# CRIPAC-DIG/GET

Measured on AMD Instinct MI355X. Metric: claim-evidence pairs/sec fwd+bwd (B=32, h=300), higher is better.
Workload: dtype f32

## Files before the change

get_amd/csrc/cell_ops.hip:

```cpp
#include "../../include/get_hip.h"
#include "gemm_batch.h"
#include "common.h"

using namespace gh;

int gh::cell_fwd_impl(int bf, float* out32, const uint64_t* bits, const float* dinv, const float* vals, const uint64_t* keep,
                                const int32_t* goff, int m_real, int m_rows,
                                const float* x, const int32_t* ids, int n, int r, int din, int h,
                                const float* w_p, const float* w_z0, const float* w_z1, const float* w_r0,
                                const float* w_r1, const float* w_h0, const float* w_h1,
                                const float* b_z0, const float* b_z1, const float* b_r0, const float* b_r1,
                                const float* b_h0, const float* b_h1,
                                float* xp, float* a, float* z, float* rr, float* rx, float* hh, float* out,
                                float drop_p, uint32_t drop_seed,
                                const float* score_w, float* score_x, float score_drop_p, uint32_t score_drop_seed,
                                gh_stream_t stream, int pad_out_dead, int* score_parts, float* xdrop) {
  hipStream_t s = (hipStream_t)stream;
  if (score_parts) *score_parts = 1;
  GH_REQUIRE(n > 0 && r > 0 && din > 0 && h > 0, "ggnn_cell_fwd: bad sizes n=%d r=%d din=%d h=%d", n, r, din, h);
  GH_REQUIRE(!bf || (din % 8 == 0 && h % 8 == 0), "ggnn_cell_fwd_bf16: needs din %% 8 == 0, h %% 8 == 0 (din=%d h=%d)", din, h);
  if (!goff) { m_real = n * r; m_rows = n * r; }
  GH_REQUIRE(m_real >= 0 && m_real <= m_rows && m_rows <= n * r, "ggnn_cell_fwd: node-compact rows %d/%d do not fit n*r=%d", m_real, m_rows, n * r);
  const int M = m_rows;
  if (M == 0) return 0;
// ... 102 lines not shown
                       score_x, score_drop_p, score_drop_seed, stream, 0, nullptr, nullptr);
}

extern "C" int gh_ggnn_cell_fwd_bf16(const uint64_t* bits, const float* dinv, const float* vals, const uint64_t* keep,
                                     const int32_t* goff, int m_real, int m_rows,
                                     const void* x, const int32_t* ids, int n, int r, int din, int h,
                                     const void* w_p, const void* w_z0, const void* w_z1, const void* w_r0,
                                     const void* w_r1, const void* w_h0, const void* w_h1,
                                     const float* b_z0, const float* b_z1, const float* b_r0, const float* b_r1,
                                     const float* b_h0, const float* b_h1,
                                     void* xp, void* a, void* z, void* rr, void* rx, void* hh, void* out, float* out32,
                                     float drop_p, uint32_t drop_seed,
                                     const float* score_w, float* score_x, float score_drop_p, uint32_t score_drop_seed,
                                     gh_stream_t stream) {
  typedef const float* cf;
  typedef float* mf;
  return cell_fwd_impl(1, out32, bits, dinv, vals, keep, goff, m_real, m_rows, (cf)x, ids, n, r, din, h, (cf)w_p, (cf)w_z0, (cf)w_z1,
                       (cf)w_r0, (cf)w_r1, (cf)w_h0, (cf)w_h1, b_z0, b_z1, b_r0, b_r1, b_h0, b_h1, (mf)xp, (mf)a, (mf)z, (mf)rr,
                       (mf)rx, (mf)hh, (mf)out, drop_p, drop_seed, score_w, score_x, score_drop_p, score_drop_seed, stream, 0, nullptr, nullptr);
}

int gh::cell_bwd_impl(int bf, const uint64_t* bits, const float* dinv, const float* vals, const uint64_t* keep,
                                const int32_t* goff, int m_real,
                                const float* x, const int32_t* ids, int n, int r, int din, int h,
                                const float* wt_p, const float* wt_z0, const float* wt_z1, const float* wt_r0,
                                const float* wt_r1, const float* wt_h0, const float* wt_h1,
                                const float* xp, const float* a, const float* z, const float* rr, const float* rx,
                                const float* hh, const float* g,
                                float* dhp, float* dzp, float* drp, float* dxp, float* da,
                                float* dx, float* dw_p, float* dw_z0, float* dw_z1, float* dw_r0, float* dw_r1,
                                float* dw_h0, float* dw_h1, float* db_z, float* db_r, float* db_h,
                                float* db_z1, float* db_r1, float* db_h1, float drop_p, uint32_t drop_seed,
                                gh_stream_t stream, gh_stream_t wstream, hipEvent_t ev_l1, hipEvent_t ev_agg,
                                int pre_done, const GateFuse* next, const float* xdrop) {
  hipStream_t s = (hipStream_t)stream;
  hipStream_t sw = wstream ? (hipStream_t)wstream : s;
  const bool two = sw != s;
  GH_REQUIRE(!two || (ev_l1 && ev_agg), "ggnn_cell_bwd: a separate weight-gradient stream needs its two events");
  GH_REQUIRE(n > 0 && r > 0 && din > 0 && h > 0, "ggnn_cell_bwd: bad sizes");
  GH_REQUIRE(!bf || (din % 8 == 0 && h % 8 == 0 && din <= h), "ggnn_cell_bwd_bf16: needs din %% 8 == 0, h %% 8 == 0, din <= h (din=%d h=%d)", din, h);
  if (!goff) m_real = n * r;
  GH_REQUIRE(m_real >= 0 && m_real <= n * r, "ggnn_cell_bwd: node-compact rows %d do not fit n*r=%d", m_real, n * r);
  GH_REQUIRE(drop_p <= 0.f || (long long)n * r * (long long)din < (1LL << 32),
             "ggnn_cell_bwd: %d rows x %d columns exceed the dropout mask's 32-bit element index", n * r, din);
  const int M = m_real;
  if (M == 0) return 0;
  if (!pre_done)
    if (int e = launch_gate_bwd_pre(g, z, hh, xp, dhp, dzp, dxp, (size_t)M * h, s, bf)) return e;
  const bool wide = bf && h % 256 == 0;
  {
    Batch b(false, M, s, wide, SITE_CELL_BWD_H, h);
    Problem p0 = gemm_problem(M, h, EPI_STORE, da, h, dhp, h, wt_h0, h, h, nullptr, bf);
    Problem p1 = gemm_problem(M, h, EPI_BWD_DRX, drp, h, dhp, h, wt_h1, h, h, nullptr, bf);
    p1.out1 = dxp; p1.in0 = xp; p1.in1 = rr;
    p0.io = bf ? 1 : 0; p1.io = bf ? 15 : 0;
    b.add(p0); b.add(p1);
    b.flush();
    GH_CHECK_HIP(b.err);
  }
  const bool cs = bf ? true : (h % 4 == 0);
  auto add_gate_wgrads = [&](Batch& b) {
    b.add(tn_problem(h, h, dw_z0, h, dzp, h, a, h, M, nullptr, bf));  if (cs) b.want_colsum(db_z, db_z1);
    b.add(tn_problem(h, h, dw_z1, h, dzp, h, xp, h, M, nullptr, bf));
    b.add(tn_problem(h, h, dw_r0, h, drp, h, a, h, M, nullptr, bf));  if (cs) b.want_colsum(db_r, db_r1);
    b.add(tn_problem(h, h, dw_r1, h, drp, h, xp, h, M, nullptr, bf));
    b.add(tn_problem(h, h, dw_h0, h, dhp, h, a, h, M, nullptr, bf));  if (cs) b.want_colsum(db_h, db_h1);
    b.add(tn_problem(h, h, dw_h1, h, dhp, h, rx, h, M, nullptr, bf));
  };
  bool colsum_done = false;
  if (two) {
    GH_CHECK_HIP(hipEventRecord(ev_l1, s));
    GH_CHECK_HIP(hipStreamWaitEvent(sw, ev_l1, 0));
    Batch b(true, M, sw);
    add_gate_wgrads(b);
    b.flush();
    GH_CHECK_HIP(b.err);
    colsum_done = b.colsum_fused && !b.colsum_missed;
    if (!colsum_done) {
      GH_REQUIRE(!bf, "ggnn_cell_bwd_bf16: the bias gradients need the split-K workspace (gh_set_workspace)");
      if (int e = launch_colsum3(dzp, drp, dhp, db_z, db_r, db_h, M, h, sw, db_z1, db_r1, db_h1)) return e;
    }
  }
// ... 32 lines not shown
    Batch b(true, M, sw);
    if (!two) add_gate_wgrads(b);
    if (bf && xdrop && drop_p > 0.f && din <= h) {
      b.add(tn_problem(h, din, dw_p, din, dxp, h, xdrop, din, M, nullptr, bf));
    } else if ((ids || drop_p > 0.f || bf) && din <= h) {
      if (int e = launch_gather_rows(x, ids, da, M, din, sw, drop_p, drop_seed, bf)) return e;
      b.add(tn_problem(h, din, dw_p, din, dxp, h, da, din, M, nullptr, bf));
    } else {
      GH_REQUIRE(drop_p == 0.f, "ggnn_cell_bwd: fused dropout needs din (%d) <= h (%d)", din, h);
      b.add(tn_problem(h, din, dw_p, din, dxp, h, x, din, M, ids));
    }
    b.flush();
    GH_CHECK_HIP(b.err);
    if (two || (b.colsum_fused && !b.colsum_missed)) return 0;
  }
  GH_REQUIRE(!bf, "ggnn_cell_bwd_bf16: the bias gradients need the split-K workspace (gh_set_workspace)");
  return launch_colsum3(dzp, drp, dhp, db_z, db_r, db_h, M, h, s, db_z1, db_r1, db_h1);
}

extern "C" int gh_ggnn_cell_bwd(const uint64_t* bits, const float* dinv, const float* vals, const uint64_t* keep,
                                const int32_t* goff, int m_real,
                                const float* x, const int32_t* ids, int n, int r, int din, int h,
                                const float* wt_p, const float* wt_z0, const float* wt_z1, const float* wt_r0,
                                const float* wt_r1, const float* wt_h0, const float* wt_h1,
                                const float* xp, const float* a, const float* z, const float* rr, const float* rx,
                                const float* hh, const float* g,
                                float* dhp, float* dzp, float* drp, float* dxp, float* da,
                                float* dx, float* dw_p, float* dw_z0, float* dw_z1, float* dw_r0, float* dw_r1,
                                float* dw_h0, float* dw_h1, float* db_z, float* db_r, float* db_h,
                                float* db_z1, float* db_r1, float* db_h1, float drop_p, uint32_t drop_seed,
                                gh_stream_t stream) {
  return cell_bwd_impl(0, bits, dinv, vals, keep, goff, m_real, x, ids, n, r, din, h, wt_p, wt_z0, wt_z1, wt_r0, wt_r1, wt_h0, wt_h1,
                       xp, a, z, rr, rx, hh, g, dhp, dzp, drp, dxp, da, dx, dw_p, dw_z0, dw_z1, dw_r0, dw_r1, dw_h0, dw_h1,
                       db_z, db_r, db_h, db_z1, db_r1, db_h1, drop_p, drop_seed, stream, nullptr, nullptr, nullptr, 0, nullptr, nullptr);
}

extern "C" int gh_ggnn_cell_bwd_bf16(const uint64_t* bits, const float* dinv, const float* vals, const uint64_t* keep,
                                     const int32_t* goff, int m_real,
                                     const void* x, const int32_t* ids, int n, int r, int din, int h,
                                     const void* wt_p, const void* wt_z0, const void* wt_z1, const void* wt_r0,
                                     const void* wt_r1, const void* wt_h0, const void* wt_h1,
                                     const void* xp, const void* a, const void* z, const void* rr, const void* rx,
                                     const void* hh, const float* g,
                                     void* dhp, void* dzp, void* drp, void* dxp, void* da,
                                     float* dx, float* dw_p, float* dw_z0, float* dw_z1, float* dw_r0, float* dw_r1,
                                     float* dw_h0, float* dw_h1, float* db_z, float* db_r, float* db_h,
                                     float* db_z1, float* db_r1, float* db_h1, float drop_p, uint32_t drop_seed,
                                     gh_stream_t stream) {
  typedef const float* cf;
  typedef float* mf;
  return cell_bwd_impl(1, bits, dinv, vals, keep, goff, m_real, (cf)x, ids, n, r, din, h, (cf)wt_p, (cf)wt_z0, (cf)wt_z1, (cf)wt_r0,
                       (cf)wt_r1, (cf)wt_h0, (cf)wt_h1, (cf)xp, (cf)a, (cf)z, (cf)rr, (cf)rx, (cf)hh, g, (mf)dhp, (mf)dzp, (mf)drp,
                       (mf)dxp, (mf)da, dx, dw_p, dw_z0, dw_z1, dw_r0, dw_r1, dw_h0, dw_h1, db_z, db_r, db_h, db_z1, db_r1,
                       db_h1, drop_p, drop_seed, stream, nullptr, nullptr, nullptr, 0, nullptr, nullptr);
}
```

get_amd/csrc/common.h:

```cpp
#pragma once
#include <hip/hip_runtime.h>
#include <stdint.h>
#include <stdio.h>
#include <stdlib.h>
#include <string.h>

namespace gh {

void set_error(const char* fmt, ...);

#define GH_CHECK_HIP(expr)                                                                  \
  do {                                                                                      \
    hipError_t _e = (expr);                                                                 \
    if (_e != hipSuccess) {                                                                 \
      gh::set_error("%s:%d: %s -> %s", __FILE__, __LINE__, #expr, hipGetErrorString(_e));   \
      return 1;                                                                             \
    }                                                                                       \
  } while (0)

#define GH_REQUIRE(cond, ...)                     \
  do {                                            \
    if (!(cond)) {                                \
      gh::set_error(__VA_ARGS__);                 \
      return 2;                                   \
// ... 68 lines not shown
int launch_att_softmax_bwd(const float* right, const float* weights, const float* g_att, const float* g_w,
                           const int32_t* goff, int m_real, int b, int l, int dr, int heads, float* de, float* dright,
                           hipStream_t s, const int32_t* rowg = nullptr, float* dw_tmp = nullptr, int* dw_written = nullptr,
                           const void* right16 = nullptr);
int launch_att_dpre(const float* de, const float* w2, const float* t, const int32_t* goff, int m_real, int b, int l,
                    int ha, int heads, float* dpre, float* du, float* dw2_part, hipStream_t s, const float* dw_in = nullptr,
                    const float* weights = nullptr, float* de_out = nullptr, void* dpre16 = nullptr,
                    long long dw_range_stride = 0, int dw_ranges = 1);

struct Workspace { float* p; size_t bytes; float* cs; size_t cs_bytes; };
Workspace workspace_for(hipStream_t s);
int gemm_mode();

struct GateFuse { const float* z; const float* hh; const float* xp; float* dhp; float* dzp; float* dxp; int bf16; };

int cell_fwd_impl(int bf, float* out32, const uint64_t* bits, const float* dinv, const float* vals, const uint64_t* keep,
                  const int32_t* goff, int m_real, int m_rows, const float* x, const int32_t* ids, int n, int r, int din, int h,
                  const float* w_p, const float* w_z0, const float* w_z1, const float* w_r0, const float* w_r1, const float* w_h0,
                  const float* w_h1, const float* b_z0, const float* b_z1, const float* b_r0, const float* b_r1, const float* b_h0,
                  const float* b_h1, float* xp, float* a, float* z, float* rr, float* rx, float* hh, float* out, float drop_p,
                  uint32_t drop_seed, const float* score_w, float* score_x, float score_drop_p, uint32_t score_drop_seed,
                  void* stream, int pad_out_dead = 0,
                  int* score_parts = nullptr,
                  float* xdrop = nullptr);
int cell_bwd_impl(int bf, const uint64_t* bits, const float* dinv, const float* vals, const uint64_t* keep, const int32_t* goff,
                  int m_real, const float* x, const int32_t* ids, int n, int r, int din, int h, const float* wt_p,
                  const float* wt_z0, const float* wt_z1, const float* wt_r0, const float* wt_r1, const float* wt_h0,
                  const float* wt_h1, const float* xp, const float* a, const float* z, const float* rr, const float* rx,
                  const float* hh, const float* g, float* dhp, float* dzp, float* drp, float* dxp, float* da, float* dx,
                  float* dw_p, float* dw_z0, float* dw_z1, float* dw_r0, float* dw_r1, float* dw_h0, float* dw_h1, float* db_z,
                  float* db_r, float* db_h, float* db_z1, float* db_r1, float* db_h1, float drop_p, uint32_t drop_seed, void* stream,
                  void* wstream, hipEvent_t ev_l1, hipEvent_t ev_agg,
                  int pre_done, const GateFuse* next,
                  const float* xdrop = nullptr);
int att_fwd_impl(const float* left, int nl, const int32_t* rowu, const float* right, const float* mask, const int32_t* goff,
                 const int32_t* rowg, int m_real, int b, int l, int xl, int dr, int ha, int heads, const float* w1, const float* w2,
                 float* u, float* t, float* e, float* weights, float* attended, hipStream_t s, int u_mode = 0,
                 const void* right16 = nullptr, const void* w1_16 = nullptr);
int att_bwd_impl(const float* left, const float* right, const int32_t* goff, int m_real, int b, int l, int xl, int dr, int ha,
                 int heads, const float* w1t, const float* w2, const float* t, const float* weights, const float* g_att,
                 const float* g_w, float* de, float* dpre, float* du, float* dleft, float* dright, float* dw1, float* dw2,
                 const int32_t* claim_offsets, int nl, float* du_c, int dleft_accumulate, hipStream_t s,
                 const int32_t* rowg = nullptr, float* dw_tmp = nullptr, const GateFuse* next = nullptr, int dleft_late = 0,
                 float* dw2_buf = nullptr, const void* right16 = nullptr, const void* w1t_16 = nullptr);
int linear2_fwd(const float* x0, int k0, const float* x1, int k1, const float* w, const float* bias, float* y, int m, int n, hipStream_t s,
                const float* w_out = nullptr, const float* b_out = nullptr, float* y_out = nullptr, int n_out = 0);
int linear2_bwd(const float* x0, int k0, const float* x1, int k1, const float* wt, const float* g, int m, int n, float* dx0,
                int dx0_accumulate, float* dx1, float* dw, float* db, hipStream_t s);

}
```

get_amd/csrc/gemm_batch.h:

```cpp
#pragma once
#include "common.h"
#include "gemm.hip.h"

namespace gh {

enum BatchSite : int {
  SITE_NONE = 0,
  SITE_CELL_ZR = 1,
  SITE_CELL_H = 2,
  SITE_CELL_BWD_H = 3,
  SITE_CELL_BWD_ZR = 4,
  SITE_CELL_BWD_DX = 5,
  SITE_ATT_BWD_DRIGHT = 6,
  SITE_CELL_PROJ = 7,
};
constexpr int NARROW_DEFAULT = 14;

long long generic_launches();

struct Batch {
  Batch(bool tn, int rows_hint, hipStream_t s, bool wide_bf16 = false, int site = SITE_NONE, int n_hint = 0);
  void add(const Problem& p);
  void flush();
  void want_colsum(float* o, float* o2) { if (L.nprob > 0) { cs_out[L.nprob - 1] = o; cs_out2[L.nprob - 1] = o2; } }

  int bm, bn;
  hipError_t err = hipSuccess;
  bool colsum_fused = false;
  bool colsum_missed = false;
  bool split_done = false;
  float* g_ws = nullptr;
  size_t g_ws_bytes = 0;
  bool narrow = false;
  long long e_block_stride = 0;

 private:
  Launch L;
  bool tn, big;
  hipStream_t s;
  int k_total = 0;
  float* cs_out[GH_MAX_PROBLEMS] = {nullptr};
  float* cs_out2[GH_MAX_PROBLEMS] = {nullptr};
  bool wide = false;
  bool wide256 = false;
  bool tn_pp = false;
  bool tn_pp_ok(const Problem& p) const;
  void reset();
  hipError_t launch_any();
  bool nt_split_plan();
};

int launch_att_finish(float* t, const float* u, const float* w2, float* e, const int32_t* urow, int M, int ha, int l, int heads, hipStream_t s);
int launch_reduce_wave(const float* parts, int n_parts, float* out, int I, int J, hipStream_t s);

inline Problem gemm_problem(int M, int N, int epi, float* C, int ldc, const float* A, int lda, const float* B, int ldb,
                            int K, const int32_t* gatherA = nullptr, int elt = 0) {
  Problem p = make_problem(M, N, epi, C, ldc);
  p.elt = elt;
  p.seg[0] = make_seg_nt(A, lda, B, ldb, K, gatherA, elt);
  return p;
}
inline void add_seg(Problem& p, const float* A, int lda, const float* B, int ldb, int K) {
  p.seg[p.nseg++] = make_seg_nt(A, lda, B, ldb, K, nullptr, p.elt);
}
inline void set_dropout(Problem& p, int mode, int ld, float drop_p, unsigned seed) {
  if (drop_p <= 0.f) return;
  p.drop_mode = mode; p.drop_ld = ld; p.drop_col0 = 0; p.drop_seed = seed;
  const double t = (double)drop_p * 4294967296.0;
  p.drop_thresh = t >= 4294967295.0 ? 4294967295u : (unsigned)t;
  p.drop_scale = 1.0f / (1.0f - drop_p);
}
inline Problem tn_problem(int I, int J, float* C, int ldc, const float* A, int lda, const float* B, int ldb, int K,
                          const int32_t* gatherB = nullptr, int elt = 0) {
  Problem p = make_problem(I, J, EPI_ATOMIC, C, ldc);
  p.seg[0] = make_seg_tn(A, lda, I, B, ldb, J, K, nullptr, gatherB);
  p.elt = elt;
  if (elt) {
    p.seg[0].vecA = ((reinterpret_cast<uintptr_t>(A) & 15) == 0) && lda % 8 == 0 && I % 8 == 0;
    p.seg[0].vecB = ((reinterpret_cast<uintptr_t>(B) & 15) == 0) && ldb % 8 == 0 && J % 8 == 0;
  }
  return p;
}

}
```

get_amd/csrc/gemm_ops.hip:

```cpp
#include "../../include/get_hip.h"
#include "gemm_batch.h"
#include "device_utils.h"
#include "gemm_nt.hip.h"
#include "gemm_tn.hip.h"
#include "gemm_tn_pp.hip.h"
#include <stdlib.h>

namespace gh {

static bool s_lds_bad(const Problem& p) { return p.seg[0].lda % 8 || p.seg[0].ldb % 8; }
static void fast_why(int rule, int prob, const Problem* p = nullptr, int seg = -1) {
  static const bool dbg = measure_env("GH_FASTOK_DEBUG", 0) != 0;
  if (!dbg) return;
  fprintf(stderr, "gemm: generic kernel (fast_ok rule %d, problem %d)\n", rule, prob);
  if (p && seg >= 0) fprintf(stderr, "   seg %d lda %d M %d N %d K %d\n", seg, p->seg[seg].lda, p->M, p->N, p->seg[seg].K);
}
static bool fast_ok(const Launch& L, bool tn) {
  for (int i = 0; i < L.nprob; ++i) {
    const Problem& p = L.p[i];
    const int ns = tn ? 1 : p.nseg;
    for (int j = 0; j < ns; ++j) {
      const Seg& s = p.seg[j];
      if (!s.vecA || !s.vecB || s.gatherB || s.K < 4) { fast_why(1, i); return false; }
      if (tn && s.gatherA) { fast_why(2, i); return false; }
// ... 294 lines not shown
      for (int u = 0; u < 8; ++u) v[u] = *reinterpret_cast<const float4*>(p + (size_t)(k + u) * it.stride);
#pragma unroll
      for (int u = 0; u < 8; ++u) { acc.x += v[u].x; acc.y += v[u].y; acc.z += v[u].z; acc.w += v[u].w; }
    }
    for (; k < it.ks; ++k) {
      const float4 v = *reinterpret_cast<const float4*>(p + (size_t)k * it.stride);
      acc.x += v.x; acc.y += v.y; acc.z += v.z; acc.w += v.w;
    }
    float* o = it.out + (size_t)i * it.ldc + j;
    o[0] += acc.x; o[1] += acc.y; o[2] += acc.z; o[3] += acc.w;
  }
}

__global__ void __launch_bounds__(256)
reduce_partials_wave_kernel(const ReduceArgs R) {
  const ReduceItem& it = R.it[blockIdx.y];
  const int J4 = it.J / 4;
  const int total = it.I * J4;
  const int e = blockIdx.x * 4 + (threadIdx.x >> 6), lane = threadIdx.x & 63;
  if (e >= total) return;
  const int i = e / J4, j = 4 * (e % J4);
  const float* p = it.ws + (size_t)i * it.J + j;
  float4 acc = make_float4(0.f, 0.f, 0.f, 0.f);
  for (int k = lane; k < it.ks; k += 64) {
    const float4 v = *reinterpret_cast<const float4*>(p + (size_t)k * it.stride);
    acc.x += v.x; acc.y += v.y; acc.z += v.z; acc.w += v.w;
  }
  for (int o = 32; o > 0; o >>= 1) {
    acc.x += __shfl_xor(acc.x, o); acc.y += __shfl_xor(acc.y, o); acc.z += __shfl_xor(acc.z, o); acc.w += __shfl_xor(acc.w, o);
  }
  if (lane == 0) {
    float* o = it.out + (size_t)i * it.ldc + j;
    o[0] += acc.x; o[1] += acc.y; o[2] += acc.z; o[3] += acc.w;
  }
}

struct FinishItem {
  const float* ws; long long stride; int ks; int M, N, epi, accumulate, ldc;
  float* C; const float* bias; const float* bias2; float* out1; const float* in0; const float* in1;
  const float* u; const float* w2; float* e; int ldu, R, heads;
  const int32_t* rowg;
};

struct FinishArgs { FinishItem it[GH_MAX_PROBLEMS]; int n; int split; };

__global__ void __launch_bounds__(256)
nt_finish_kernel(const FinishArgs F) {
  const FinishItem& it = F.it[blockIdx.y];
  const int lane = threadIdx.x & 63, wave = threadIdx.x >> 6;
  const bool split = F.split != 0;
  const int row = split ? (int)blockIdx.x : (int)blockIdx.x * 4 + wave;
  if (row >= it.M) return;
  const int N4 = it.N / 4;
  __shared__ float4 part[3][64];
  int kb = 0, ke = it.ks;
  if (split) { const int kq = (it.ks + 3) / 4; kb = wave * kq; ke = min(it.ks, kb + kq); }
  float pe[8];
#pragma unroll
  for (int c = 0; c < 8; ++c) pe[c] = 0.f;
  for (int c0 = 0; c0 < N4; c0 += 64) {
    const int c4 = c0 + lane;
    const int col = 4 * c4;
    float4 v = make_float4(0.f, 0.f, 0.f, 0.f);
    if (c4 < N4 && kb < ke) {
      const float* p = it.ws + (size_t)row * it.N + col;
      for (int k0 = kb; k0 < ke; k0 += 8) {
// ... 317 lines not shown
    q.split_stride = (long long)q.M * q.N;
    w += (size_t)ks * q.M * q.N;
    if (q.M > max_m) max_m = q.M;
  }
  L.ksplit = ks;
  L.kchunk = ct * 16;
  hipError_t e = launch_any();
  if (e != hipSuccess) err = e;
  F.split = (ks >= 16 && max_m <= 8192) ? 1 : 0;
  hipLaunchKernelGGL(nt_finish_kernel, dim3(F.split ? max_m : (max_m + 3) / 4, F.n), dim3(256), 0, s, F);
  split_done = true;
  e = hipGetLastError();
  if (e != hipSuccess) err = e;
  reset();
  return true;
}

int launch_att_finish(float* t, const float* u, const float* w2, float* e, const int32_t* urow, int M, int ha, int l, int heads, hipStream_t s) {
  FinishArgs F;
  F.n = 1; F.split = 0;
  F.it[0] = FinishItem{t, 0, 1, M, ha, EPI_ATT, 0, ha, t, nullptr, nullptr, nullptr, nullptr, nullptr, u, w2, e, ha, l, heads, urow};
  hipLaunchKernelGGL(nt_finish_kernel, dim3((M + 3) / 4, 1), dim3(256), 0, s, F);
  GH_LAUNCH_CHECK();
  return 0;
}
int launch_reduce_wave(const float* parts, int n_parts, float* out, int I, int J, hipStream_t s) {
  ReduceArgs R;
  R.n = 1;
  R.it[0] = ReduceItem{parts, out, I, J, J, n_parts, (long long)I * J};
  hipLaunchKernelGGL(reduce_partials_wave_kernel, dim3((I * (J / 4) + 3) / 4, 1), dim3(256), 0, s, R);
  GH_LAUNCH_CHECK();
  return 0;
}

}

using namespace gh;

extern "C" int gh_set_gemm_mode(int mode) {
  GH_REQUIRE(mode >= 0 && mode <= 3, "set_gemm_mode: %d is not 0 (fp32), 1 (bf16 operands in the big NT/NN GEMMs), 2 (fp32x3) or 3 (fp32x3, pre-split weights)", mode);
  g_gemm_mode = mode;
  return 0;
}

extern "C" int gh_weights_changed(void) {
  std::lock_guard<std::mutex> lk(g_x3_mu);
  ++g_x3_epoch;
  return 0;
}

extern "C" int gh_fp32x3_refresh(gh_stream_t stream) {
  std::lock_guard<std::mutex> lk(g_x3_mu);
  if (g_x3.empty()) return 0;
  std::vector<X3Item> items;
  items.reserve(g_x3.size());
  for (auto& kv : g_x3) {
    items.push_back(X3Item{(const float*)kv.first.b, kv.second.img, kv.first.N, kv.first.ldb, kv.first.K, kv.second.pitch});
    kv.second.epoch = g_x3_epoch;
  }
  x3p_split(items.data(), (int)items.size(), (hipStream_t)stream);
  GH_CHECK_HIP(hipGetLastError());
  return 0;
}

extern "C" int gh_fp32x3_clear(void) {
  std::lock_guard<std::mutex> lk(g_x3_mu);
// ... 40 lines not shown
```

get_amd/csrc/model_ops.hip:

```cpp
#include "../../include/get_hip.h"
#include "common.h"
#include <mutex>
#include <unordered_map>

namespace gh {

struct Dims {
  int B, B1, L, R, n, D, H, hw, he, C, cs, as, Xl, Xa, Dre, E, W;
  bool compact;
  int Mr, Mt, M1, Mq;
  bool bf;
  bool att16;
  bool fuse_scorer;
};
struct CellBuf { int64_t xp, a, z, rr, rx, hh, out, out32, xdrop; };
struct FwdBuf {
  int64_t offsets, pair2claim, has, lens_eff, rowc, maskf_p;
  CellBuf q, c1, c2;
  int64_t q_repr, score_x, score, keep;
  int64_t uw, tw, ew, ww, avg, new_left;
  int64_t right_e, mask_e, ue, te, ee, we, att_e, y0, phi;
  int64_t total;
  int64_t obs_total;
};
// ... 271 lines not shown
  P->phi = f.phi; P->word_w = f.ww; P->evd_w = f.we; P->score = f.score; P->keep = f.keep;
  return 0;
}

extern "C" int gh_get_struct_sizes(int64_t* out) {
  GH_REQUIRE(out, "get_struct_sizes: NULL");
  out[0] = sizeof(gh_get_model); out[1] = sizeof(gh_get_batch); out[2] = sizeof(gh_get_plan); out[3] = sizeof(gh_cell_params);
  out[4] = sizeof(gh_cell_bf16);
  return 0;
}

#define GH_TRY(expr) do { if (int _rc = (expr)) return _rc; } while (0)

static inline const int32_t* I32(const float* A, int64_t off) { return reinterpret_cast<const int32_t*>(A + off); }
static inline int32_t* I32(float* A, int64_t off) { return reinterpret_cast<int32_t*>(A + off); }

static int cell_fwd(const gh_cell_params& c, const gh_cell_bf16* c16, const CellBuf& cb, float* A, const uint64_t* bits, const float* dinv,
                    const float* vals, const uint64_t* keep, const int32_t* goff, int m_real, int m_rows, const float* x, const int32_t* ids,
                    int n, int r, int din, int h, float drop_p, uint32_t seed, const float* score_w, float* score_x, float sdrop,
                    uint32_t sseed, hipStream_t s, int pad_out_dead = 0, int* score_parts = nullptr) {
  typedef const float* cf;
  if (c16)
    return cell_fwd_impl(1, cb.out32 >= 0 ? A + cb.out32 : nullptr, bits, dinv, vals, keep, goff, m_real, m_rows, x, ids, n, r, din, h, (cf)c16->w_p, (cf)c16->w_z0,
                         (cf)c16->w_z1, (cf)c16->w_r0, (cf)c16->w_r1, (cf)c16->w_h0, (cf)c16->w_h1, c.b_z0, c.b_z1, c.b_r0, c.b_r1, c.b_h0,
                         c.b_h1, A + cb.xp, A + cb.a, A + cb.z, A + cb.rr, A + cb.rx, A + cb.hh, A + cb.out, drop_p, seed, score_w, score_x,
                         sdrop, sseed, (void*)s, 0, score_parts, cb.xdrop >= 0 ? A + cb.xdrop : nullptr);
  return cell_fwd_impl(0, nullptr, bits, dinv, vals, keep, goff, m_real, m_rows, x, ids, n, r, din, h, c.w_p, c.w_z0, c.w_z1, c.w_r0,
                       c.w_r1, c.w_h0, c.w_h1, c.b_z0, c.b_z1, c.b_r0, c.b_r1, c.b_h0, c.b_h1, A + cb.xp, A + cb.a, A + cb.z,
                       A + cb.rr, A + cb.rx, A + cb.hh, A + cb.out, drop_p, seed, score_w, score_x, sdrop, sseed, (void*)s, pad_out_dead);
}
static int cell_bwd(const gh_cell_params& c, const gh_cell_bf16* c16, const CellBuf& cb, const float* A, const uint64_t* bits, const float* dinv,
                    const float* vals, const uint64_t* keep, const int32_t* goff, int m_real, const float* x, const int32_t* ids, int n,
                    int r, int din, int h, const float* g, float* W, const int64_t* sc, float* dx, float drop_p, uint32_t seed,
                    hipStream_t s, int pre_done = 0, const GateFuse* next = nullptr) {
  GH_REQUIRE(c.dw_p && c.db_z0 && c.db_z1, "get_backward: a cell's gradient outputs are missing");
  if (c16) {
    typedef const float* cf;
    GH_REQUIRE(c16->wt_p && c16->wt_z0 && c16->wt_z1 && c16->wt_r0 && c16->wt_r1 && c16->wt_h0 && c16->wt_h1,
               "get_backward: storage = 1 needs the bf16 twins of the cells' transposed weights (gh_weights_refresh)");
    return cell_bwd_impl(1, bits, dinv, vals, keep, goff, m_real, x, ids, n, r, din, h, (cf)c16->wt_p, (cf)c16->wt_z0, (cf)c16->wt_z1,
                         (cf)c16->wt_r0, (cf)c16->wt_r1, (cf)c16->wt_h0, (cf)c16->wt_h1, A + cb.xp, A + cb.a, A + cb.z, A + cb.rr,
                         A + cb.rx, A + cb.hh, g, W + sc[0], W + sc[1], W + sc[2], W + sc[3], W + sc[4], dx, c.dw_p, c.dw_z0, c.dw_z1,
                         c.dw_r0, c.dw_r1, c.dw_h0, c.dw_h1, c.db_z0, c.db_r0, c.db_h0, c.db_z1, c.db_r1, c.db_h1, drop_p, seed, (void*)s,
                         nullptr, nullptr, nullptr, pre_done, next, cb.xdrop >= 0 ? A + cb.xdrop : nullptr);
  }
  GH_REQUIRE(c.wt_p, "get_backward: a cell's transposes are missing");
  return cell_bwd_impl(0, bits, dinv, vals, keep, goff, m_real, x, ids, n, r, din, h, c.wt_p, c.wt_z0, c.wt_z1, c.wt_r0, c.wt_r1,
                       c.wt_h0, c.wt_h1, A + cb.xp, A + cb.a, A + cb.z, A + cb.rr, A + cb.rx, A + cb.hh, g, W + sc[0], W + sc[1],
                       W + sc[2], W + sc[3], W + sc[4], dx, c.dw_p, c.dw_z0, c.dw_z1, c.dw_r0, c.dw_r1, c.dw_h0, c.dw_h1, c.db_z0,
                       c.db_r0, c.db_h0, c.db_z1, c.db_r1, c.db_h1, drop_p, seed, (void*)s, nullptr, nullptr, nullptr, pre_done, next);
}

extern "C" int gh_get_forward(const gh_get_model* Mo, const gh_get_batch* Ba, float* A, float* O, gh_stream_t stream, gh_stream_t side_stream) {
  Dims d; FwdBuf f; BwdBuf w;
  GH_TRY(layout(Mo, Ba, d, f, w));
  GH_REQUIRE(A && (reinterpret_cast<uintptr_t>(A) & 255) == 0, "get_forward: the arena must be 256-byte aligned");
  GH_REQUIRE(O && (reinterpret_cast<uintptr_t>(O) & 255) == 0, "get_forward: the observables buffer must be 256-byte aligned");
  GH_REQUIRE(Ba->q_ids && Ba->q_lens && Ba->q_bits && (Ba->q_dinv || Ba->q_vals) && Ba->d_ids && Ba->d_bits && (Ba->d_dinv || Ba->d_vals) &&
             Ba->counts && Ba->document, "get_forward: a batch tensor is missing (ids, lens, packed graphs, counts, document)");
  GH_REQUIRE(Ba->q_lens_kind >= 0 && Ba->q_lens_kind <= 2, "get_forward: q_lens_kind %d not in {0,1,2}", Ba->q_lens_kind);
  GH_REQUIRE(d.as == 0 || Ba->doc_sources, "get_forward: article-source ids are missing");
  GH_REQUIRE(d.cs == 0 || Ba->query_sources, "get_forward: claim-source ids are missing");
  GH_REQUIRE(Mo->embedding && Mo->scorer_w && Mo->scorer_gate && Mo->out0_w && Mo->out1_w, "get_forward: missing model tensors");
  GH_REQUIRE((d.cs == 0) == (Mo->claim_src_table == nullptr) && (d.as == 0) == (Mo->article_src_table == nullptr),
             "get_forward: source tables and their widths must come together");
  GH_REQUIRE(d.cs == 0 || Mo->claim_src_rows > 0, "get_forward: claim_src_rows must give the claim-source table's row count");
  GH_REQUIRE(d.as == 0 || Mo->article_src_rows > 0, "get_forward: article_src_rows must give the article-source table's row count");
  GH_REQUIRE(Ba->drop_claim >= 0.f && Ba->drop_claim < 1.f && Ba->drop_gnn >= 0.f && Ba->drop_gnn < 1.f, "get_forward: dropout p not in [0,1)");
  hipStream_t s = (hipStream_t)stream, ss = side_stream ? (hipStream_t)side_stream : s;
  DevEvents ev;
  GH_TRY(get_events(ev));
  const int H = d.H;
  if (d.B <= 1024) {
    const int nthr = d.Mr > d.B1 ? d.Mr : d.B1;
    const dim3 grid((nthr + 255) / 256);
    const int32_t* rg = d.compact ? Ba->rowg : nullptr;
    float* mp = d.compact ? nullptr : A + f.maskf_p;
    if (Ba->q_lens_kind == 0)
      hipLaunchKernelGGL(seg_rows_kernel<float>, grid, dim3(256), 0, s, Ba->counts, d.B, d.B1, rg, d.R, d.Mr, I32(A, f.offsets), I32(A, f.pair2claim),
                         A + f.has, I32(A, f.rowc), Ba->d_ids, mp, (const float*)Ba->q_lens, A + f.lens_eff);
    else if (Ba->q_lens_kind == 1)
      hipLaunchKernelGGL(seg_rows_kernel<int32_t>, grid, dim3(256), 0, s, Ba->counts, d.B, d.B1, rg, d.R, d.Mr, I32(A, f.offsets), I32(A, f.pair2claim),
                         A + f.has, I32(A, f.rowc), Ba->d_ids, mp, (const int32_t*)Ba->q_lens, A + f.lens_eff);
// ... 111 lines not shown
    GH_TRY(stream_after(ss, s, ev.ev[2]));
    GH_TRY(linear2_bwd(A + f.new_left, d.Xl, A + f.att_e, d.Dre * d.he, Mo->out0_wt, Wb + w.d_y0, d.B, H, nullptr, 0, nullptr,
                       Mo->d_out0_w, Mo->d_out0_b, ss));
    GH_TRY(att_bwd_impl(A + f.new_left, A + f.right_e, nullptr, 0, d.B, d.n, d.Xl, d.Dre, H, d.he, Mo->att_evd.w1t, Mo->att_evd.w2, A + f.te,
                        O + f.we, Wb + w.d_att_e, g_evd_w, Wb + w.de_e, Wb + w.dpre_e, Wb + w.du_e, Wb + w.d_new_left, Wb + w.dright_e,
                        nullptr, Mo->att_evd.dw2, nullptr, d.B, nullptr, 1, s, nullptr, (d.Dre + 511) / 512 <= 16 ? Wb + w.dw_e : nullptr, nullptr, 1,
                        Wb + w.dw2p_e));
    GH_TRY(stream_after(ss, s, ev.ev[3]));
    GH_TRY(att_bwd_impl(A + f.new_left, A + f.right_e, nullptr, 0, d.B, d.n, d.Xl, d.Dre, H, d.he, Mo->att_evd.w1t, Mo->att_evd.w2, A + f.te,
                        O + f.we, Wb + w.d_att_e, g_evd_w, Wb + w.de_e, Wb + w.dpre_e, Wb + w.du_e, Wb + w.d_new_left, nullptr, Mo->att_evd.dw1,
                        Mo->att_evd.dw2, nullptr, d.B, nullptr, 1, ss, nullptr, nullptr, nullptr, 1, Wb + w.dw2p_e));
    if (d.cs > 0) {
      if (Ba->query_sources_i64)
        hipLaunchKernelGGL(left_assemble_bwd_kernel<int64_t>, dim3(1), dim3(256), 0, ss, Wb + w.d_new_left, (const int64_t*)Ba->query_sources,
                           A + f.has, Wb + w.d_q, Mo->d_claim_src_table, d.B, d.cs, H, Mo->claim_src_rows);
      else
        hipLaunchKernelGGL(left_assemble_bwd_kernel<int32_t>, dim3(1), dim3(256), 0, ss, Wb + w.d_new_left, (const int32_t*)Ba->query_sources,
                           A + f.has, Wb + w.d_q, Mo->d_claim_src_table, d.B, d.cs, H, Mo->claim_src_rows);
      GH_LAUNCH_CHECK();
    }
    GH_TRY(gh_evd_assemble_bwd(Wb + w.dright_e, I32(A, f.offsets), d.as > 0 ? Ba->doc_sources : nullptr, Ba->doc_sources_i64, Mo->article_src_rows, d.B, d.n, d.Xa,
                               d.as, Wb + w.d_avg, d.as > 0 ? Mo->d_article_src_table : nullptr, (void*)s));
    GH_TRY(att_bwd_impl(A + f.q_repr, f.c2.out32 >= 0 ? A + f.c2.out32 : nullptr, goff, d.Mr, d.B1, d.R, H, H, H, d.hw, Mo->att_word.w1t, Mo->att_word.w2, A + f.tw,
                        O + f.ww, Wb + w.d_avg, g_word_w, Wb + w.de_w, Wb + w.dpre_w, Wb + w.du_w, Wb + w.d_q, Wb + w.g2, nullptr,
                        Mo->att_word.dw2, I32(A, f.offsets), d.B, Wb + w.du_c, 1, s, d.compact ? Ba->rowg : nullptr, Wb + w.dw_w,
                        fuse_gate ? &gf2 : nullptr, 1, Wb + w.dw2p_w, att_r16, att_w1t16));
    GH_TRY(stream_after(ss, s, ev.ev[4]));
    GH_TRY(att_bwd_impl(A + f.q_repr, f.c2.out32 >= 0 ? A + f.c2.out32 : nullptr, goff, d.Mr, d.B1, d.R, H, H, H, d.hw, Mo->att_word.w1t, Mo->att_word.w2, A + f.tw,
                        O + f.ww, Wb + w.d_avg, g_word_w, Wb + w.de_w, Wb + w.dpre_w, Wb + w.du_w, Wb + w.d_q, nullptr, Mo->att_word.dw1,
                        Mo->att_word.dw2, I32(A, f.offsets), d.B, Wb + w.du_c, 1, ss, nullptr, nullptr, nullptr, 1, Wb + w.dw2p_w, att_r16,
                        att_w1t16));
    GH_TRY(gh_masked_mean_bwd(Wb + w.d_q, Ba->q_ids, A + f.lens_eff, Wb + w.d_qhid, d.B, d.L, H, (void*)ss));
    GH_TRY(cell_bwd(Mo->claim, nullptr, f.q, A, Ba->q_bits, Ba->q_dinv, Ba->q_vals, nullptr, nullptr, 0, Mo->embedding, Ba->q_ids, d.B, d.L, d.D, H,
                    Wb + w.d_qhid, Wb, w.qs, nullptr, Ba->drop_claim, Ba->seed_claim, ss));
    if (fuse_gate)
      GH_TRY(cell_bwd(Mo->cell2, c16_2, f.c2, A, Ba->d_bits, Ba->d_dinv, Ba->d_vals, keep, goff, d.Mr, A + f.c1.out, nullptr, d.B1, d.R, H, H,
                      Wb + w.g2, Wb, w.sc2, nullptr, Ba->drop_gnn, Ba->seed_cell2, s, 1, &gf1));
    else
      GH_TRY(cell_bwd(Mo->cell2, c16_2, f.c2, A, Ba->d_bits, Ba->d_dinv, Ba->d_vals, keep, goff, d.Mr, A + f.c1.out, nullptr, d.B1, d.R, H, H,
                      Wb + w.g2, Wb, w.sc2, Wb + w.dx2, Ba->drop_gnn, Ba->seed_cell2, s, 0, nullptr));
  }
  if (phase != 1) {
    if (fuse_gate)
      GH_TRY(cell_bwd(Mo->cell1, c16_1, f.c1, A, Ba->d_bits, Ba->d_dinv, Ba->d_vals, nullptr, goff, d.Mr, table1, ids1, d.B1, d.R, d.D, H,
                      nullptr, Wb, w.sc1, nullptr, Ba->drop_gnn, Ba->seed_cell1, s, 1, nullptr));
    else
      GH_TRY(cell_bwd(Mo->cell1, c16_1, f.c1, A, Ba->d_bits, Ba->d_dinv, Ba->d_vals, nullptr, goff, d.Mr, table1, ids1, d.B1, d.R, d.D, H,
                      Wb + w.dx2, Wb, w.sc1, nullptr, Ba->drop_gnn, Ba->seed_cell1, s, 0, nullptr));
    GH_TRY(stream_after(s, ss, ev.ev[5]));
  }
  return 0;
}

extern "C" int gh_cross_entropy(const float* phi, const int64_t* labels, int b, int c, float* loss, float* dphi, gh_stream_t stream) {
  GH_REQUIRE(b > 0 && c > 0 && phi && labels && loss && dphi, "cross_entropy: bad arguments");
  unsigned int* cl = clamp_counter();
  GH_REQUIRE(cl, "cross_entropy: cannot allocate the clamp counter");
  hipLaunchKernelGGL(cross_entropy_kernel, dim3(1), dim3(256), 0, (hipStream_t)stream, phi, labels, b, c, loss, dphi, cl);
  GH_LAUNCH_CHECK();
  return 0;
}

extern "C" int gh_get_prepare(const int32_t* claim_tokens, const int32_t* claim_len, int b, int l,
                              const int32_t* evd_tokens, const int32_t* evd_len, int b1, int r, int window,
                              int32_t* q_ids, int32_t* q_n, uint64_t* q_bits, float* q_dinv,
                              int32_t* d_ids, int32_t* d_n, uint64_t* d_bits, float* d_dinv,
                              int m_real, int32_t* goff, int32_t* rowg, int32_t* src, int32_t* cids, float* maskf,
                              const int64_t* slot, int32_t* document, gh_stream_t stream) {
  if (b > 0 && b1 > 0) {
    GH_TRY(launch_graph_build2(claim_tokens, claim_len, b, l, q_ids, q_n, q_bits, q_dinv, evd_tokens, evd_len, b1, r, d_ids, d_n, d_bits,
                               d_dinv, window, (hipStream_t)stream));
  } else {
    GH_TRY(gh_graph_build(claim_tokens, claim_len, b, l, window, q_ids, q_n, q_bits, q_dinv, stream));
    GH_TRY(gh_graph_build(evd_tokens, evd_len, b1, r, window, d_ids, d_n, d_bits, d_dinv, stream));
  }
  bool scattered = false;
  if (m_real >= 0 && b1 > 0) {
    GH_TRY(launch_ragged_plan(d_n, d_ids, b1, r, goff, rowg, src, cids, maskf, slot, document, (hipStream_t)stream, &scattered));
  }
  if (slot && document && b1 > 0 && !scattered) {
    hipLaunchKernelGGL(document_scatter_kernel, dim3(b1), dim3(256), 0, (hipStream_t)stream, d_ids, slot, document, r);
// ... 5 lines not shown
```

Before: 165,000.

## Reassociate first-cell weight gradients through input projection when no input gradient is needed

When the cell's input gradient is not required (first GGNN cell, fp32), the backward no longer forms the projected-input activations' gradients at full hidden width. It computes small h×din products of the gate gradients against the raw or aggregated input, then assembles all weight gradients, including the projection weight, with a new multi-term NN accumulate MFMA kernel. This reassociation is meant to cut GEMM FLOPs and memory traffic since din is smaller than h. It adds scratch use at the workspace tail, an extra spmm over the input, and a new kernel whose reduction order differs from the original.

```diff
diff --git a/get_amd/csrc/cell_ops.hip b/get_amd/csrc/cell_ops.hip
--- a/get_amd/csrc/cell_ops.hip
+++ b/get_amd/csrc/cell_ops.hip
@@ -158,7 +158,7 @@
                                 float* dw_h0, float* dw_h1, float* db_z, float* db_r, float* db_h,
                                 float* db_z1, float* db_r1, float* db_h1, float drop_p, uint32_t drop_seed,
                                 gh_stream_t stream, gh_stream_t wstream, hipEvent_t ev_l1, hipEvent_t ev_agg,
-                                int pre_done, const GateFuse* next, const float* xdrop) {
+                                int pre_done, const GateFuse* next, const float* xdrop, float* ybuf, int nodx_ok) {
   hipStream_t s = (hipStream_t)stream;
   hipStream_t sw = wstream ? (hipStream_t)wstream : s;
   const bool two = sw != s;
@@ -174,6 +174,86 @@
   if (!pre_done)
     if (int e = launch_gate_bwd_pre(g, z, hh, xp, dhp, dzp, dxp, (size_t)M * h, s, bf)) return e;
   const bool wide = bf && h % 256 == 0;
+  const size_t ts_floats = 5 * (size_t)h * (size_t)din;
+  const Workspace wsp = workspace_for(s);
+  const bool nodx = nodx_ok && !dx && !next && !bf && !two && din <= h && din % 4 == 0 && h % 4 == 0 && wsp.p != nullptr &&
+                    (reinterpret_cast<uintptr_t>(wsp.p) & 15) == 0 && wsp.bytes / 2 >= ts_floats * sizeof(float);
+  if (nodx) {
+    const size_t hd = (size_t)h * (size_t)din;
+    float* ts = wsp.p + wsp.bytes / sizeof(float) - ts_floats;
+    float *t_z = ts, *t_r = ts + hd, *t_h = ts + 2 * hd, *s_z = ts + 3 * hd, *s_r = ts + 4 * hd;
+    const size_t ws_left = wsp.bytes - ts_floats * sizeof(float);
+    {
+      Batch b(false, M, s, false, SITE_CELL_BWD_H, h);
+      Problem p1 = gemm_problem(M, h, EPI_BWD_DRX, drp, h, dhp, h, wt_h1, h, h);
+      p1.out1 = dxp; p1.in0 = xp; p1.in1 = rr;
+      b.add(p1);
+      b.flush();
+      GH_CHECK_HIP(b.err);
+    }
+    const float* X = x;
+    if (ids || drop_p > 0.f) {
+      if (int e = launch_gather_rows(x, ids, da, M, din, s, drop_p, drop_seed, 0)) return e;
+      X = da;
+    }
+    bool cs_ok = false;
+    auto add_s = [&](Batch& b) {
+      b.add(tn_problem(h, din, s_z, din, dzp, h, X, din, M));  if (!ybuf) b.want_colsum(db_z, db_z1);
+      b.add(tn_problem(h, din, s_r, din, drp, h, X, din, M));  if (!ybuf) b.want_colsum(db_r, db_r1);
+      b.add(tn_problem(h, h, dw_h1, h, dhp, h, rx, h, M));     if (!ybuf) b.want_colsum(db_h, db_h1);
+      b.add(tn_problem(h, din, dw_p, din, dxp, h, X, din, M));
+    };
+    if (ybuf) {
+      ZeroFill zf = {ts, (long long)ts_floats, nullptr, 0};
+      bool zf_done = false;
+      if (int e = launch_spmm(bits, dinv, vals, keep, goff, m_real, X, ybuf, n, r, din, 0, 0, s, 0, &zf, &zf_done)) return e;
+      if (!zf_done) GH_CHECK_HIP(hipMemsetAsync(ts, 0, ts_floats * sizeof(float), s));
+      Batch b(true, M, s);
+      b.g_ws_bytes = ws_left;
+      b.add(tn_problem(h, din, t_z, din, dzp, h, ybuf, din, M));  b.want_colsum(db_z, db_z1);
+      b.add(tn_problem(h, din, t_r, din, drp, h, ybuf, din, M));  b.want_colsum(db_r, db_r1);
+      b.add(tn_problem(h, din, t_h, din, dhp, h, ybuf, din, M));  b.want_colsum(db_h, db_h1);
+      add_s(b);
+      b.flush();
+      GH_CHECK_HIP(b.err);
+      cs_ok = b.colsum_fused && !b.colsum_missed;
+    } else {
+      GH_CHECK_HIP(hipMemsetAsync(ts, 0, ts_floats * sizeof(float), s));
+      Batch b(true, M, s);
+      b.g_ws_bytes = ws_left;
+      add_s(b);
+      b.flush();
+      GH_CHECK_HIP(b.err);
+      cs_ok = b.colsum_fused && !b.colsum_missed;
+      if (int e = launch_spmm(bits, dinv, vals, keep, goff, m_real, X, dxp, n, r, din, 0, 0, s, 0)) return e;
+      Batch b2(true, M, s);
+      b2.g_ws_bytes = ws_left;
+      b2.add(tn_problem(h, din, t_z, din, dzp, h, dxp, din, M));
+      b2.add(tn_problem(h, din, t_r, din, drp, h, dxp, din, M));
+      b2.add(tn_problem(h, din, t_h, din, dhp, h, dxp, din, M));
+      b2.flush();
+      GH_CHECK_HIP(b2.err);
+    }
+    NnArgs R;
+    memset(&R, 0, sizeof(R));
+    R.n = 6;
+    NnItem& ip = R.it[0];
+    ip.C = dw_p; ip.I = h; ip.J = din; ip.ldc = din;
+    nn_add_term(ip, wt_z0, h, t_z, din, h);
+    nn_add_term(ip, wt_r0, h, t_r, din, h);
+    nn_add_term(ip, wt_h0, h, t_h, din, h);
+    nn_add_term(ip, wt_z1, h, s_z, din, h);
+    nn_add_term(ip, wt_r1, h, s_r, din, h);
+    float* const dwg[5] = {dw_z0, dw_r0, dw_h0, dw_z1, dw_r1};
+    for (int i = 0; i < 5; ++i) {
+      NnItem& it = R.it[1 + i];
+      it.C = dwg[i]; it.I = h; it.J = h; it.ldc = h;
+      nn_add_term(it, ts + i * hd, din, wt_p, h, din);
+    }
+    if (int e = launch_nn_accumulate(R, s)) return e;
+    if (cs_ok) return 0;
+    return launch_colsum3(dzp, drp, dhp, db_z, db_r, db_h, M, h, s, db_z1, db_r1, db_h1);
+  }
   {
     Batch b(false, M, s, wide, SITE_CELL_BWD_H, h);
     Problem p0 = gemm_problem(M, h, EPI_STORE, da, h, dhp, h, wt_h0, h, h, nullptr, bf);
@@ -272,7 +352,7 @@
                                 gh_stream_t stream) {
   return cell_bwd_impl(0, bits, dinv, vals, keep, goff, m_real, x, ids, n, r, din, h, wt_p, wt_z0, wt_z1, wt_r0, wt_r1, wt_h0, wt_h1,
                        xp, a, z, rr, rx, hh, g, dhp, dzp, drp, dxp, da, dx, dw_p, dw_z0, dw_z1, dw_r0, dw_r1, dw_h0, dw_h1,
-                       db_z, db_r, db_h, db_z1, db_r1, db_h1, drop_p, drop_seed, stream, nullptr, nullptr, nullptr, 0, nullptr, nullptr);
+                       db_z, db_r, db_h, db_z1, db_r1, db_h1, drop_p, drop_seed, stream, nullptr, nullptr, nullptr, 0, nullptr, nullptr, nullptr, 1);
 }
 
 extern "C" int gh_ggnn_cell_bwd_bf16(const uint64_t* bits, const float* dinv, const float* vals, const uint64_t* keep,
@@ -292,5 +372,5 @@
   return cell_bwd_impl(1, bits, dinv, vals, keep, goff, m_real, (cf)x, ids, n, r, din, h, (cf)wt_p, (cf)wt_z0, (cf)wt_z1, (cf)wt_r0,
                        (cf)wt_r1, (cf)wt_h0, (cf)wt_h1, (cf)xp, (cf)a, (cf)z, (cf)rr, (cf)rx, (cf)hh, g, (mf)dhp, (mf)dzp, (mf)drp,
                        (mf)dxp, (mf)da, dx, dw_p, dw_z0, dw_z1, dw_r0, dw_r1, dw_h0, dw_h1, db_z, db_r, db_h, db_z1, db_r1,
-                       db_h1, drop_p, drop_seed, stream, nullptr, nullptr, nullptr, 0, nullptr, nullptr);
-}
+                       db_h1, drop_p, drop_seed, stream, nullptr, nullptr, nullptr, 0, nullptr, nullptr, nullptr, 1);
+}
diff --git a/get_amd/csrc/common.h b/get_amd/csrc/common.h
--- a/get_amd/csrc/common.h
+++ b/get_amd/csrc/common.h
@@ -124,7 +124,9 @@
                   float* db_r, float* db_h, float* db_z1, float* db_r1, float* db_h1, float drop_p, uint32_t drop_seed, void* stream,
                   void* wstream, hipEvent_t ev_l1, hipEvent_t ev_agg,
                   int pre_done, const GateFuse* next,
-                  const float* xdrop = nullptr);
+                  const float* xdrop = nullptr,
+                  float* ybuf = nullptr,
+                  int nodx_ok = 1);
 int att_fwd_impl(const float* left, int nl, const int32_t* rowu, const float* right, const float* mask, const int32_t* goff,
                  const int32_t* rowg, int m_real, int b, int l, int xl, int dr, int ha, int heads, const float* w1, const float* w2,
                  float* u, float* t, float* e, float* weights, float* attended, hipStream_t s, int u_mode = 0,
diff --git a/get_amd/csrc/gemm_batch.h b/get_amd/csrc/gemm_batch.h
--- a/get_amd/csrc/gemm_batch.h
+++ b/get_amd/csrc/gemm_batch.h
@@ -52,6 +52,14 @@
 
 int launch_att_finish(float* t, const float* u, const float* w2, float* e, const int32_t* urow, int M, int ha, int l, int heads, hipStream_t s);
 int launch_reduce_wave(const float* parts, int n_parts, float* out, int I, int J, hipStream_t s);
+constexpr int NN_MAX_TERMS = 5, NN_MAX_ITEMS = 6;
+struct NnTerm { const float* A; const float* B; int lda, ldb, K, vec; };
+struct NnItem { float* C; int I, J, ldc, nterm, tile0; NnTerm t[NN_MAX_TERMS]; };
+struct NnArgs { NnItem it[NN_MAX_ITEMS]; int n; };
+inline void nn_add_term(NnItem& it, const float* A, int lda, const float* B, int ldb, int K) {
+  it.t[it.nterm++] = NnTerm{A, B, lda, ldb, K, 0};
+}
+int launch_nn_accumulate(NnArgs& R, hipStream_t s);
 
 inline Problem gemm_problem(int M, int N, int epi, float* C, int ldc, const float* A, int lda, const float* B, int ldb,
                             int K, const int32_t* gatherA = nullptr, int elt = 0) {
diff --git a/get_amd/csrc/gemm_ops.hip b/get_amd/csrc/gemm_ops.hip
--- a/get_amd/csrc/gemm_ops.hip
+++ b/get_amd/csrc/gemm_ops.hip
@@ -350,6 +350,95 @@
   if (lane == 0) {
     float* o = it.out + (size_t)i * it.ldc + j;
     o[0] += acc.x; o[1] += acc.y; o[2] += acc.z; o[3] += acc.w;
+  }
+}
+
+constexpr int NN_T = 32, NN_K = 16, NN_WAVES = 8;
+__global__ void __launch_bounds__(64 * NN_WAVES)
+nn_accumulate_kernel(const NnArgs R_byval) {
+  (void)R_byval;
+  const GH_KARG NnArgs& R = *(const GH_KARG NnArgs*)__builtin_amdgcn_kernarg_segment_ptr();
+  __shared__ float red[NN_WAVES][NN_T][NN_T];
+  int item = 0;
+  while (item + 1 < R.n && (int)blockIdx.x >= R.it[item + 1].tile0) ++item;
+  const GH_KARG NnItem& it = R.it[item];
+  const int I = it.I, J = it.J;
+  const int tiles_j = (J + NN_T - 1) / NN_T;
+  const int tile = (int)blockIdx.x - it.tile0;
+  const int i0 = (tile / tiles_j) * NN_T, j0 = (tile % tiles_j) * NN_T;
+  const int w = threadIdx.x >> 6, lane = threadIdx.x & 63;
+  const int l15 = lane & 15, q = lane >> 4;
+  int total = 0;
+  for (int t = 0; t < it.nterm; ++t) total += (it.t[t].K + NN_K - 1) / NN_K;
+  int row[2], col[2];
+#pragma unroll
+  for (int m = 0; m < 2; ++m) {
+    row[m] = i0 + m * 16 + l15; if (row[m] > I - 1) row[m] = I - 1;
+    col[m] = j0 + m * 16 + l15; if (col[m] > J - 1) col[m] = J - 1;
+  }
+  f32x4 acc[2][2];
+#pragma unroll
+  for (int mi = 0; mi < 2; ++mi)
+#pragma unroll
+    for (int ni = 0; ni < 2; ++ni) acc[mi][ni] = f32x4{0.f, 0.f, 0.f, 0.f};
+  int t = 0, base = 0;
+  for (int c = w; c < total; c += NN_WAVES) {
+    for (;;) {
+      const int nc = (it.t[t].K + NN_K - 1) / NN_K;
+      if (c < base + nc) break;
+      base += nc; ++t;
+    }
+    const GH_KARG NnTerm& tm = it.t[t];
+    const float* A = tm.A;
+    const float* B = tm.B;
+    const int K = tm.K, lda = tm.lda, ldb = tm.ldb;
+    const int kk = (c - base) * NN_K + 4 * q;
+    float av[2][4], bv[2][4];
+#pragma unroll
+    for (int mi = 0; mi < 2; ++mi) {
+      const float* ap = A + (size_t)row[mi] * lda + kk;
+      if (tm.vec) {
+        const float4 v = kk < K ? *reinterpret_cast<const float4*>(ap) : make_float4(0.f, 0.f, 0.f, 0.f);
+        av[mi][0] = v.x; av[mi][1] = v.y; av[mi][2] = v.z; av[mi][3] = v.w;
+      } else {
+#pragma unroll
+        for (int s = 0; s < 4; ++s) av[mi][s] = kk + s < K ? ap[s] : 0.f;
+      }
+    }
+#pragma unroll
+    for (int ni = 0; ni < 2; ++ni)
+#pragma unroll
+      for (int s = 0; s < 4; ++s) bv[ni][s] = kk + s < K ? B[(size_t)(kk + s) * ldb + col[ni]] : 0.f;
+#pragma unroll
+    for (int s = 0; s < 4; ++s)
+#pragma unroll
+      for (int mi = 0; mi < 2; ++mi)
+#pragma unroll
+        for (int ni = 0; ni < 2; ++ni)
+          acc[mi][ni] = __builtin_amdgcn_mfma_f32_16x16x4f32(av[mi][s], bv[ni][s], acc[mi][ni], 0, 0, 0);
+  }
+#pragma unroll
+  for (int mi = 0; mi < 2; ++mi)
+#pragma unroll
+    for (int ni = 0; ni < 2; ++ni)
+#pragma unroll
+      for (int reg = 0; reg < 4; ++reg) red[w][mi * 16 + 4 * q + reg][ni * 16 + l15] = acc[mi][ni][reg];
+  __syncthreads();
+  if (threadIdx.x >= NN_T * NN_T / 4) return;
+  const int ri = threadIdx.x >> 3, rj = 4 * (threadIdx.x & 7);
+  float4 sum = *reinterpret_cast<const float4*>(&red[0][ri][rj]);
+#pragma unroll
+  for (int v = 1; v < NN_WAVES; ++v) {
+    const float4 p = *reinterpret_cast<const float4*>(&red[v][ri][rj]);
+    sum.x += p.x; sum.y += p.y; sum.z += p.z; sum.w += p.w;
+  }
+  const int gi = i0 + ri, gj = j0 + rj;
+  if (gi < I) {
+    float* o = it.C + (size_t)gi * it.ldc + gj;
+    const float sv[4] = {sum.x, sum.y, sum.z, sum.w};
+#pragma unroll
+    for (int e = 0; e < 4; ++e)
+      if (gj + e < J) o[e] += sv[e];
   }
 }
 
@@ -733,6 +822,23 @@
   GH_LAUNCH_CHECK();
   return 0;
 }
+int launch_nn_accumulate(NnArgs& R, hipStream_t s) {
+  GH_REQUIRE(R.n > 0 && R.n <= NN_MAX_ITEMS, "nn_accumulate: %d items", R.n);
+  int tiles = 0;
+  for (int i = 0; i < R.n; ++i) {
+    NnItem& it = R.it[i];
+    GH_REQUIRE(it.C && it.I > 0 && it.J > 0 && it.ldc >= it.J && it.nterm > 0 && it.nterm <= NN_MAX_TERMS, "nn_accumulate: bad item %d", i);
+    for (int t = 0; t < it.nterm; ++t)
+      GH_REQUIRE(it.t[t].A && it.t[t].B && it.t[t].K > 0 && it.t[t].lda >= it.t[t].K && it.t[t].ldb >= it.J, "nn_accumulate: bad term %d of item %d", t, i);
+    for (int t = 0; t < it.nterm; ++t)
+      it.t[t].vec = (reinterpret_cast<uintptr_t>(it.t[t].A) & 15) == 0 && it.t[t].lda % 4 == 0 && it.t[t].K % 4 == 0;
+    it.tile0 = tiles;
+    tiles += ((it.I + NN_T - 1) / NN_T) * ((it.J + NN_T - 1) / NN_T);
+  }
+  hipLaunchKernelGGL(nn_accumulate_kernel, dim3(tiles), dim3(64 * NN_WAVES), 0, s, R);
+  GH_LAUNCH_CHECK();
+  return 0;
+}
 
 }
 
diff --git a/get_amd/csrc/model_ops.hip b/get_amd/csrc/model_ops.hip
--- a/get_amd/csrc/model_ops.hip
+++ b/get_amd/csrc/model_ops.hip
@@ -327,7 +327,7 @@
 static int cell_bwd(const gh_cell_params& c, const gh_cell_bf16* c16, const CellBuf& cb, const float* A, const uint64_t* bits, const float* dinv,
                     const float* vals, const uint64_t* keep, const int32_t* goff, int m_real, const float* x, const int32_t* ids, int n,
                     int r, int din, int h, const float* g, float* W, const int64_t* sc, float* dx, float drop_p, uint32_t seed,
-                    hipStream_t s, int pre_done = 0, const GateFuse* next = nullptr) {
+                    hipStream_t s, int pre_done = 0, const GateFuse* next = nullptr, float* ybuf = nullptr, int nodx_ok = 1) {
   GH_REQUIRE(c.dw_p && c.db_z0 && c.db_z1, "get_backward: a cell's gradient outputs are missing");
   if (c16) {
     typedef const float* cf;
@@ -343,7 +343,8 @@
   return cell_bwd_impl(0, bits, dinv, vals, keep, goff, m_real, x, ids, n, r, din, h, c.wt_p, c.wt_z0, c.wt_z1, c.wt_r0, c.wt_r1,
                        c.wt_h0, c.wt_h1, A + cb.xp, A + cb.a, A + cb.z, A + cb.rr, A + cb.rx, A + cb.hh, g, W + sc[0], W + sc[1],
                        W + sc[2], W + sc[3], W + sc[4], dx, c.dw_p, c.dw_z0, c.dw_z1, c.dw_r0, c.dw_r1, c.dw_h0, c.dw_h1, c.db_z0,
-                       c.db_r0, c.db_h0, c.db_z1, c.db_r1, c.db_h1, drop_p, seed, (void*)s, nullptr, nullptr, nullptr, pre_done, next);
+                       c.db_r0, c.db_h0, c.db_z1, c.db_r1, c.db_h1, drop_p, seed, (void*)s, nullptr, nullptr, nullptr, pre_done, next,
+                       nullptr, ybuf, nodx_ok);
 }
 
 extern "C" int gh_get_forward(const gh_get_model* Mo, const gh_get_batch* Ba, float* A, float* O, gh_stream_t stream, gh_stream_t side_stream) {
@@ -521,7 +522,7 @@
                         att_w1t16));
     GH_TRY(gh_masked_mean_bwd(Wb + w.d_q, Ba->q_ids, A + f.lens_eff, Wb + w.d_qhid, d.B, d.L, H, (void*)ss));
     GH_TRY(cell_bwd(Mo->claim, nullptr, f.q, A, Ba->q_bits, Ba->q_dinv, Ba->q_vals, nullptr, nullptr, 0, Mo->embedding, Ba->q_ids, d.B, d.L, d.D, H,
-                    Wb + w.d_qhid, Wb, w.qs, nullptr, Ba->drop_claim, Ba->seed_claim, ss));
+                    Wb + w.d_qhid, Wb, w.qs, nullptr, Ba->drop_claim, Ba->seed_claim, ss, 0, nullptr, nullptr, 0));
     if (fuse_gate)
       GH_TRY(cell_bwd(Mo->cell2, c16_2, f.c2, A, Ba->d_bits, Ba->d_dinv, Ba->d_vals, keep, goff, d.Mr, A + f.c1.out, nullptr, d.B1, d.R, H, H,
                       Wb + w.g2, Wb, w.sc2, nullptr, Ba->drop_gnn, Ba->seed_cell2, s, 1, &gf1));
@@ -530,12 +531,13 @@
                       Wb + w.g2, Wb, w.sc2, Wb + w.dx2, Ba->drop_gnn, Ba->seed_cell2, s, 0, nullptr));
   }
   if (phase != 1) {
+    float* const y1 = d.bf ? nullptr : Wb + w.sc2[4];
     if (fuse_gate)
       GH_TRY(cell_bwd(Mo->cell1, c16_1, f.c1, A, Ba->d_bits, Ba->d_dinv, Ba->d_vals, nullptr, goff, d.Mr, table1, ids1, d.B1, d.R, d.D, H,
-                      nullptr, Wb, w.sc1, nullptr, Ba->drop_gnn, Ba->seed_cell1, s, 1, nullptr));
+                      nullptr, Wb, w.sc1, nullptr, Ba->drop_gnn, Ba->seed_cell1, s, 1, nullptr, y1));
     else
       GH_TRY(cell_bwd(Mo->cell1, c16_1, f.c1, A, Ba->d_bits, Ba->d_dinv, Ba->d_vals, nullptr, goff, d.Mr, table1, ids1, d.B1, d.R, d.D, H,
-                      Wb + w.dx2, Wb, w.sc1, nullptr, Ba->drop_gnn, Ba->seed_cell1, s, 0, nullptr));
+                      Wb + w.dx2, Wb, w.sc1, nullptr, Ba->drop_gnn, Ba->seed_cell1, s, 0, nullptr, y1));
     GH_TRY(stream_after(s, ss, ev.ev[5]));
   }
   return 0;
```

Measured after the change: 180,800 (median of 6 runs). 9.6% higher.
